# kotoba-tech/kotoba-whisper

Hardware: AMD Instinct MI355X
Metric: audio-seconds/sec (RTF) whisper-large-v3 30s@bs32 (higher is better)
Workload: dtype bf16; 1 GPU; config 3: whisper-large-v3 greedy generate, 30 s clips, log-mel on GPU; model=openai/whisper-large-v3, global_batch=32, per_gpu_batch=32, max_length=128, seq_len=1500, parallelism=dp1

## Files before the change

kotoba-whisper_amd/csrc/decproj.h:

```cpp
#pragma once
#include "declin_tile.h"
#include "kw_common.h"

#ifndef KW_PROJ_STAMP
#define KW_PROJ_STAMP(slot)
#endif

namespace {

constexpr int PROJ_KTM = 5;
constexpr int PROJ_NV = 8;
constexpr int PROJ_SCRATCH = 16384 + 2048 + 256;

struct ProjArgs {
  const bf16_t* x;
  int64_t ldx;
  int M, K, N;
  float ln_eps;
  const float* colsum;
  const bf16x8* W;
  const float* bias;
  float scale;
  int scale_cols;
  int* fault;
};

__host__ __device__ __forceinline__ bool proj_shape_ok(int64_t M, int64_t K) {
  return M >= 1 && M <= 32 && K % 32 == 0 && K / 32 <= PROJ_NV * PROJ_KTM;
}

template <bool ONESHOT>
__device__ __forceinline__ void proj_publish_granules(const ProjArgs& a, int cg, char* scratch,
                                                      unsigned long long* gran) {
  f32x4(*red)[2][64] = reinterpret_cast<f32x4(*)[2][64]>(scratch);
  float(*rpart)[32][2] = reinterpret_cast<float(*)[32][2]>(scratch + 16384);
  float(*rstat)[2] = reinterpret_cast<float(*)[2]>(scratch + 16384 + 2048);
  const int lane = threadIdx.x & 63, wave = __builtin_amdgcn_readfirstlane(threadIdx.x >> 6);
  const int M = a.M, nkt = a.K >> 5;
  const int nv = (nkt + PROJ_KTM - 1) / PROJ_KTM;
  KW_PROJ_STAMP(0);
  const bool xtiled = a.ldx == KW_LD_TILED;
  const int xks = xtiled ? (M > 16 ? 1024 : 512) : 32;
  const bf16_t* x0 = xtiled ? a.x + lane * 8 : a.x + (int64_t)min(lane & 15, M - 1) * a.ldx + (lane >> 4) * 8;
  const bf16_t* x1 = xtiled ? x0 + (M > 16 ? 512 : 0) : a.x + (int64_t)min(16 + (lane & 15), M - 1) * a.ldx + (lane >> 4) * 8;
  const int n_e = min(cg * 16 + (lane & 15), a.N - 1);
  const float ebias = a.bias ? a.bias[n_e] : 0.f;
  const float ecsum = a.colsum[n_e];
  const int fault = __hip_atomic_load(a.fault, __ATOMIC_RELAXED, __HIP_MEMORY_SCOPE_AGENT);
  bf16x8 wv[2][PROJ_KTM];
#pragma unroll
  for (int r = 0; r < 2; ++r) {
    const int v = min(wave + 4 * r, nv - 1);
    const int kt0 = (nkt * v) / nv, kt1 = (nkt * (v + 1)) / nv;
    const int ktl = max(kt1 - 1, kt0);
    if (wave + 4 * r < nv) {
#pragma unroll
      for (int u = 0; u < PROJ_KTM; ++u)
        wv[r][u] = __builtin_nontemporal_load(a.W + ((int64_t)cg * nkt + min(kt0 + u, ktl)) * 64 + lane);
    }
  }
  bf16x8 av[2][2][PROJ_KTM];
  auto load_a = [&](int r) {
    const int v = min(wave + 4 * r, nv - 1);
    const int kt0 = (nkt * v) / nv, kt1 = (nkt * (v + 1)) / nv;
    const int ktl = max(kt1 - 1, kt0);
#pragma unroll
    for (int u = 0; u < PROJ_KTM; ++u) {
      const int kt = min(kt0 + u, ktl);
      av[r][0][u] = *reinterpret_cast<const bf16x8*>(x0 + kt * xks);
      av[r][1][u] = *reinterpret_cast<const bf16x8*>(x1 + kt * xks);
    }
  };
  load_a(0);
  if (ONESHOT && wave + 4 < nv) load_a(1);
#pragma unroll
  for (int r = 0; r < 2; ++r) {
    const int v = wave + 4 * r;
    if (v >= nv) break;
    const int kt0 = (nkt * v) / nv, kt1 = (nkt * (v + 1)) / nv;
    const bf16x8* w = wv[r];
    if (!ONESHOT && r) load_a(1);
    const bf16x8(&a0)[PROJ_KTM] = av[r][0];
    const bf16x8(&a1)[PROJ_KTM] = av[r][1];
    f32x4 c0 = f32x4{0.f, 0.f, 0.f, 0.f}, c1 = c0;
#pragma unroll
    for (int u = 0; u < PROJ_KTM; ++u)
      if (kt0 + u < kt1) {
        c0 = __builtin_amdgcn_mfma_f32_16x16x32_bf16(a0[u], w[u], c0, 0, 0, 0);
        c1 = __builtin_amdgcn_mfma_f32_16x16x32_bf16(a1[u], w[u], c1, 0, 0, 0);
      }
    ln_row_partials<PROJ_KTM, true>(a0, a1, kt0, kt1, lane, rpart[v]);
    red[v][0][lane] = c0;
    red[v][1][lane] = c1;
  }
  KW_PROJ_STAMP(1);
  __syncthreads();
  if (wave >= 2) return;
  const int hh = wave;
  f32x4 c = red[0][hh][lane];
  for (int v = 1; v < nv; ++v) c += red[v][hh][lane];
  if (lane < 16) ln_finish_row(rpart, nv, 16 * hh + lane, a.K, a.ln_eps, rstat);
  wave_lds_sync();
  const int n = cg * 16 + (lane & 15);
  const bool drop = cg == 0 && fault != 0;
  if (drop && wave == 0 && lane == 0) __hip_atomic_store(a.fault, 0, __ATOMIC_RELAXED, __HIP_MEMORY_SCOPE_AGENT);
#pragma unroll
  for (int r = 0; r < 4; ++r) {
    const int m = 16 * hh + 4 * (lane >> 4) + r;
    float v = c[r];
    v = ln_fold(v, rstat[m][0], rstat[m][1], ecsum);
    v += ebias;
    if (n < a.scale_cols) v *= a.scale;
    const uint32_t mine = f2bf(v);
    const uint32_t other = (uint32_t)__builtin_amdgcn_update_dpp(0, (int)mine, 0xB1, 0xF, 0xF, false);
    if ((lane & 1) == 0 && m < M && n < a.N && !drop)
      __hip_atomic_store(gran + (int64_t)m * (a.N / 2) + (n >> 1), (1ull << 32) | (mine | (other << 16)),
                         __ATOMIC_RELAXED, __HIP_MEMORY_SCOPE_AGENT);
  }
  KW_PROJ_STAMP(2);
}

}
```

kotoba-whisper_amd/csrc/qkvself.hip:

```cpp
#include "attn_common.h"
#include "decproj.h"

#ifndef KW_QS_STAMP
#define KW_QS_STAMP(slot)
#endif

namespace {

constexpr int QS_PAIRS = 2;
constexpr int QS_MAX_LEN = 256;

struct QSP {
  const bf16_t* x;
  int64_t ldx;
  float ln_eps;
  const float* ln_colsum;
  const bf16x8* W;
  const float* bias;
  float scale;
  int M, d, H, n_lin;
  bf16_t* kc;
  bf16_t* vc;
  int t_max;
  const int32_t* cur_len;
  unsigned long long* gran;
  int* err;
  bf16_t* out;
  int out_t;
};

__global__ __launch_bounds__(256) __attribute__((amdgpu_waves_per_eu(3))) void qkv_self_kernel(QSP p) {
  __shared__ __attribute__((aligned(16))) char scratch[PROJ_SCRATCH];
  __shared__ float ared[QS_PAIRS][2][64];
  __shared__ float astat[QS_PAIRS][4];
  __shared__ uint32_t stage[QS_PAIRS][96];
  const int d = p.d, H = p.H, M = p.M;
  if ((int)blockIdx.x < p.n_lin) {
    proj_publish_granules<true>(ProjArgs{p.x, p.ldx, M, d, 3 * d, p.ln_eps, p.ln_colsum, p.W, p.bias, p.scale, d, p.err + 1},
                          blockIdx.x, scratch, p.gran);
    return;
  }
  KW_QS_STAMP(4);
  const int tid = threadIdx.x, lane = tid & 63, wave = __builtin_amdgcn_readfirstlane(tid >> 6);
  const int ps = wave >> 1, pw = wave & 1, ptid = tid & 127;
  const int L = *p.cur_len;
  const bool len_ok = L >= 1 && L <= QS_MAX_LEN && L <= p.t_max;
  const int Lc = len_ok ? L : 1;
  const int p0 = Lc - 1;

  const int pair = ((int)blockIdx.x - p.n_lin) * QS_PAIRS + ps;
  const bool has_pair = pair < M * H;
  const int b = has_pair ? pair / H : 0, h = has_pair ? pair - (pair / H) * H : 0;
  const int sub = lane & 7, slot = pw * 8 + (lane >> 3);
  bf16_t* kb = p.kc + ((int64_t)b * H + h) * p.t_max * HD;
  bf16_t* vb = p.vc + ((int64_t)b * H + h) * p.t_max * HD;
  const int nj0 = min((Lc + 15) >> 4, 8), nj1 = max(min((Lc - 128 + 15) >> 4, 8), 0);
  u32x4 kr[8], vr[8];
  if (has_pair) {
#pragma unroll
    for (int j = 0; j < 8; ++j)
      if (j < nj0) kr[j] = ld_row8<bf16_t>(kb + (int64_t)min(slot + 16 * j, p0) * HD + sub * 8).u[0];
#pragma unroll
    for (int j = 0; j < 8; ++j)
      if (j < nj0) vr[j] = ld_row8<bf16_t>(vb + (int64_t)min(slot + 16 * j, p0) * HD + sub * 8).u[0];
  }

  if (has_pair && ptid < 96) {
    const int part = ptid >> 5, c = ptid & 31;
    unsigned long long* g = p.gran + (int64_t)b * (3 * d / 2) + part * (d / 2) + h * 32 + c;
    unsigned long long x = 0;
    int it = 0;
    for (;; ++it) {
      x = __hip_atomic_load(g, __ATOMIC_RELAXED, __HIP_MEMORY_SCOPE_AGENT);
      if ((x >> 32) == 1ull || it >= XG_SPIN_LIMIT) break;
      __builtin_amdgcn_s_sleep(KW_POLL_SLEEP);
    }
    if ((x >> 32) != 1ull || !len_ok) {
      x = 0x7fc07fc0ull;
      __hip_atomic_store(p.err, 1, __ATOMIC_RELAXED, __HIP_MEMORY_SCOPE_AGENT);
    }
    stage[ps][ptid] = (uint32_t)x;
    __hip_atomic_store(g, 0ull, __ATOMIC_RELAXED, __HIP_MEMORY_SCOPE_AGENT);
  }
  __syncthreads();
  KW_QS_STAMP(5);
  if (has_pair) {
    const uint32_t* st = stage[ps];
    const u32x4 qraw = {st[sub * 4], st[sub * 4 + 1], st[sub * 4 + 2], st[sub * 4 + 3]};
    const u32x4 knew = {st[32 + sub * 4], st[32 + sub * 4 + 1], st[32 + sub * 4 + 2], st[32 + sub * 4 + 3]};
    const u32x4 vnew = {st[64 + sub * 4], st[64 + sub * 4 + 1], st[64 + sub * 4 + 2], st[64 + sub * 4 + 3]};
    float ql[8];
    query_log2(qraw, ql);
    const int pn = p0 >> 7, jn = (p0 & 127) >> 4, sn = p0 & 15;
#pragma unroll
    for (int j = 0; j < 8; ++j)
      if (pn == 0 && j == jn && slot == sn) {
        kr[j] = knew;
        vr[j] = vnew;
      }
    float mw, lw, acc[8];
    wave_row_bf16<16>(ql, kr, vr, 0, Lc, slot, nj0, mw, lw, acc);
    if (nj1 > 0) {
#pragma unroll
      for (int j = 0; j < 8; ++j)
        if (j < nj1) kr[j] = ld_row8<bf16_t>(kb + (int64_t)min(128 + slot + 16 * j, p0 - 1) * HD + sub * 8).u[0];
#pragma unroll
      for (int j = 0; j < 8; ++j)
        if (j < nj1) vr[j] = ld_row8<bf16_t>(vb + (int64_t)min(128 + slot + 16 * j, p0 - 1) * HD + sub * 8).u[0];
#pragma unroll
      for (int j = 0; j < 8; ++j)
        if (pn == 1 && j == jn && slot == sn) {
          kr[j] = knew;
          vr[j] = vnew;
        }
      float m1, l1, a1[8];
      wave_row_bf16<16>(ql, kr, vr, 128, Lc, slot, nj1, m1, l1, a1);
      const float mn = fmaxf(mw, m1);
      const float f0 = __builtin_amdgcn_exp2f(mw - mn), f1 = __builtin_amdgcn_exp2f(m1 - mn);
      lw = fmaf(lw, f0, l1 * f1);
#pragma unroll
      for (int i = 0; i < 8; ++i) acc[i] = fmaf(acc[i], f0, a1[i] * f1);
      mw = mn;
    }
    if (slot == sn && len_ok) {
      *reinterpret_cast<u32x4*>(kb + (int64_t)p0 * HD + sub * 8) = knew;
      *reinterpret_cast<u32x4*>(vb + (int64_t)p0 * HD + sub * 8) = vnew;
    }
    if (lane < 8) {
#pragma unroll
      for (int i = 0; i < 8; ++i) ared[ps][pw][lane * 8 + i] = acc[i];
    }
    if (lane == 0) {
      astat[ps][pw] = mw;
      astat[ps][2 + pw] = lw;
    }
  }
  KW_QS_STAMP(6);
  __syncthreads();
  if (has_pair && ptid < HD) {
    const float* st = astat[ps];
    const float m = fmaxf(st[0], st[1]);
    const float f0 = __builtin_amdgcn_exp2f(st[0] - m), f1 = __builtin_amdgcn_exp2f(st[1] - m);
    const float l = fmaf(st[2], f0, st[3] * f1);
    const float o = fmaf(ared[ps][0][ptid], f0, ared[ps][1][ptid] * f1);
    p.out[p.out_t ? kw_tiled_off(b, h * HD + ptid, p.out_t) : (int64_t)b * d + h * HD + ptid] = f2bf(o / l);
  }
  KW_QS_STAMP(7);
}

size_t qs_gran_bytes(int64_t M, int64_t d) { return (size_t)M * (size_t)(3 * d / 2) * sizeof(unsigned long long); }

bool qs_shape_ok(int64_t M, int64_t d, int64_t H) {
  return proj_shape_ok(M, d) && H >= 1 && d == 64 * H;
}

}

extern "C" size_t kw_dec_qkv_self_workspace(int64_t M, int64_t d) {
  return (M >= 1 && d > 0) ? qs_gran_bytes(M, d) + 64 : 0;
}

extern "C" size_t kw_dec_qkv_self_status_offset(int64_t M, int64_t d) {
  return (M >= 1 && d > 0) ? qs_gran_bytes(M, d) : 0;
}

extern "C" int kw_dec_qkv_self_supported(int64_t M, int64_t d, int64_t H) {
  return qs_shape_ok(M, d, H) ? 1 : 0;
}

extern "C" int kw_dec_qkv_self(const kw_dec_qkv_self_args* a, kw_stream_t stream) {
  if (!a || !a->x || !a->W || !a->ln_colsum || !a->k_cache || !a->v_cache || !a->cur_len || !a->out || !a->workspace)
    return kw_set_error_msg(KW_EINVAL, "kw_dec_qkv_self: null pointer");
  if (!qs_shape_ok(a->M, a->d, a->H) || (a->ldx != KW_LD_TILED && (a->ldx < a->d || a->ldx % 8)) || (uintptr_t)a->x % 16 || a->t_max < 1 ||
      a->t_max > 4096)
    return kw_set_error_msg(KW_EINVAL, "kw_dec_qkv_self: M <= 32 rows, d = 64 H <= 1280, ldx % 8 == 0, 16-B aligned x");
  if (a->ws_bytes < kw_dec_qkv_self_workspace(a->M, a->d))
    return kw_set_error_msg(KW_EINVAL, "kw_dec_qkv_self: needs a zero-filled workspace of kw_dec_qkv_self_workspace()");
  QSP p;
  p.x = reinterpret_cast<const bf16_t*>(a->x);
  p.ldx = a->ldx;
  p.ln_eps = a->ln_eps;
  p.ln_colsum = a->ln_colsum;
  p.W = reinterpret_cast<const bf16x8*>(a->W);
  p.bias = a->bias;
  p.scale = a->scale;
  p.M = (int)a->M;
  p.d = (int)a->d;
  p.H = (int)a->H;
  p.n_lin = (int)(3 * a->d / 16);
  p.kc = reinterpret_cast<bf16_t*>(a->k_cache);
  p.vc = reinterpret_cast<bf16_t*>(a->v_cache);
  p.t_max = (int)a->t_max;
  p.cur_len = a->cur_len;
  p.gran = reinterpret_cast<unsigned long long*>(a->workspace);
  p.err = reinterpret_cast<int*>(reinterpret_cast<char*>(a->workspace) + qs_gran_bytes(a->M, a->d));
  p.out = reinterpret_cast<bf16_t*>(a->out);
  p.out_t = a->ldx == KW_LD_TILED ? (int)((a->M + 15) / 16) : 0;
  const int grid = p.n_lin + (int)((a->M * a->H + QS_PAIRS - 1) / QS_PAIRS);
  hipLaunchKernelGGL(qkv_self_kernel, dim3((unsigned)grid), dim3(256), 0, (hipStream_t)stream, p);
  KW_CHECK_LAUNCH();
  return KW_OK;
}
```

Baseline: 2391 audio-s/s.

## Widen qkv_self blocks to 8 waves and stagger attention KV loads

Doubles the attention pairs per block to four, giving 512-thread blocks. Adds a projection variant in which each of eight waves handles one K-slice in a single pass, instead of four waves looping over two slices. Attention blocks now sleep briefly before loading the KV cache, so the projection blocks' weight streaming gets memory bandwidth first. The aim is less serialization inside projection blocks and less contention with the attention prologue. The costs are a fixed sleep on the attention path, lower occupancy from the larger blocks, and tuning that depends on timing.

```diff
diff --git a/kotoba-whisper_amd/csrc/decproj.h b/kotoba-whisper_amd/csrc/decproj.h
--- a/kotoba-whisper_amd/csrc/decproj.h
+++ b/kotoba-whisper_amd/csrc/decproj.h
@@ -120,4 +120,59 @@
   KW_PROJ_STAMP(2);
 }
 
+__device__ __forceinline__ void proj_publish_granules_w8(const ProjArgs& a, int cg, char* scratch,
+                                                         unsigned long long* gran) {
+  f32x4(*red)[2][64] = reinterpret_cast<f32x4(*)[2][64]>(scratch);
+  float(*rpart)[32][2] = reinterpret_cast<float(*)[32][2]>(scratch + 16384);
+  float(*rstat)[2] = reinterpret_cast<float(*)[2]>(scratch + 16384 + 2048);
+  const int lane = threadIdx.x & 63, wave = __builtin_amdgcn_readfirstlane(threadIdx.x >> 6);
+  const int M = a.M, nkt = a.K >> 5;
+  const int nv = (nkt + PROJ_KTM - 1) / PROJ_KTM;
+  KW_PROJ_STAMP(0);
+  const int n_e = min(cg * 16 + (lane & 15), a.N - 1);
+  if (wave < nv) {
+    const int kt0 = (nkt * wave) / nv, kt1 = (nkt * (wave + 1)) / nv;
+    const int ktl = max(kt1 - 1, kt0);
+    bf16x8 w[1][PROJ_KTM], a0[PROJ_KTM], a1[PROJ_KTM];
+    load_w_frags<PROJ_KTM, 1, true>(a.W, cg, nkt, kt0, ktl, lane, w);
+    if (a.ldx == KW_LD_TILED)
+      load_x_frags_tiled<PROJ_KTM, true>(a.x, M > 16 ? 2 : 1, kt0, ktl, lane, a0, a1);
+    else
+      load_x_frags_rows<PROJ_KTM, true>(a.x, a.ldx, M, kt0, ktl, lane, a0, a1);
+    f32x4 c0[1], c1[1];
+    mfma_tile<PROJ_KTM, 1, true>(a0, a1, w, kt0, kt1, c0, c1);
+    ln_row_partials<PROJ_KTM, true>(a0, a1, kt0, kt1, lane, rpart[wave]);
+    red[wave][0][lane] = c0[0];
+    red[wave][1][lane] = c1[0];
+  }
+  const float ebias = a.bias ? a.bias[n_e] : 0.f;
+  const float ecsum = a.colsum[n_e];
+  const int fault = __hip_atomic_load(a.fault, __ATOMIC_RELAXED, __HIP_MEMORY_SCOPE_AGENT);
+  KW_PROJ_STAMP(1);
+  __syncthreads();
+  if (wave >= 2) return;
+  const int hh = wave;
+  f32x4 c = red[0][hh][lane];
+  for (int v = 1; v < nv; ++v) c += red[v][hh][lane];
+  if (lane < 16) ln_finish_row(rpart, nv, 16 * hh + lane, a.K, a.ln_eps, rstat);
+  wave_lds_sync();
+  const int n = cg * 16 + (lane & 15);
+  const bool drop = cg == 0 && fault != 0;
+  if (drop && wave == 0 && lane == 0) __hip_atomic_store(a.fault, 0, __ATOMIC_RELAXED, __HIP_MEMORY_SCOPE_AGENT);
+#pragma unroll
+  for (int r = 0; r < 4; ++r) {
+    const int m = 16 * hh + 4 * (lane >> 4) + r;
+    float v = c[r];
+    v = ln_fold(v, rstat[m][0], rstat[m][1], ecsum);
+    v += ebias;
+    if (n < a.scale_cols) v *= a.scale;
+    const uint32_t mine = f2bf(v);
+    const uint32_t other = (uint32_t)__builtin_amdgcn_update_dpp(0, (int)mine, 0xB1, 0xF, 0xF, false);
+    if ((lane & 1) == 0 && m < M && n < a.N && !drop)
+      __hip_atomic_store(gran + (int64_t)m * (a.N / 2) + (n >> 1), (1ull << 32) | (mine | (other << 16)),
+                         __ATOMIC_RELAXED, __HIP_MEMORY_SCOPE_AGENT);
+  }
+  KW_PROJ_STAMP(2);
 }
+
+}
diff --git a/kotoba-whisper_amd/csrc/qkvself.hip b/kotoba-whisper_amd/csrc/qkvself.hip
--- a/kotoba-whisper_amd/csrc/qkvself.hip
+++ b/kotoba-whisper_amd/csrc/qkvself.hip
@@ -5,9 +5,13 @@
 #define KW_QS_STAMP(slot)
 #endif
 
+#ifndef KW_QS_KV_DELAY
+#define KW_QS_KV_DELAY 48
+#endif
+
 namespace {
 
-constexpr int QS_PAIRS = 2;
+constexpr int QS_PAIRS = 4;
 constexpr int QS_MAX_LEN = 256;
 
 struct QSP {
@@ -29,15 +33,15 @@
   int out_t;
 };
 
-__global__ __launch_bounds__(256) __attribute__((amdgpu_waves_per_eu(3))) void qkv_self_kernel(QSP p) {
+__global__ __launch_bounds__(64 * 2 * QS_PAIRS) __attribute__((amdgpu_waves_per_eu(4))) void qkv_self_kernel(QSP p) {
   __shared__ __attribute__((aligned(16))) char scratch[PROJ_SCRATCH];
   __shared__ float ared[QS_PAIRS][2][64];
   __shared__ float astat[QS_PAIRS][4];
   __shared__ uint32_t stage[QS_PAIRS][96];
   const int d = p.d, H = p.H, M = p.M;
   if ((int)blockIdx.x < p.n_lin) {
-    proj_publish_granules<true>(ProjArgs{p.x, p.ldx, M, d, 3 * d, p.ln_eps, p.ln_colsum, p.W, p.bias, p.scale, d, p.err + 1},
-                          blockIdx.x, scratch, p.gran);
+    proj_publish_granules_w8(ProjArgs{p.x, p.ldx, M, d, 3 * d, p.ln_eps, p.ln_colsum, p.W, p.bias, p.scale, d, p.err + 1},
+                             blockIdx.x, scratch, p.gran);
     return;
   }
   KW_QS_STAMP(4);
@@ -56,6 +60,7 @@
   bf16_t* vb = p.vc + ((int64_t)b * H + h) * p.t_max * HD;
   const int nj0 = min((Lc + 15) >> 4, 8), nj1 = max(min((Lc - 128 + 15) >> 4, 8), 0);
   u32x4 kr[8], vr[8];
+  if (KW_QS_KV_DELAY > 0) __builtin_amdgcn_s_sleep(KW_QS_KV_DELAY);
   if (has_pair) {
 #pragma unroll
     for (int j = 0; j < 8; ++j)
@@ -197,7 +202,7 @@
   p.out = reinterpret_cast<bf16_t*>(a->out);
   p.out_t = a->ldx == KW_LD_TILED ? (int)((a->M + 15) / 16) : 0;
   const int grid = p.n_lin + (int)((a->M * a->H + QS_PAIRS - 1) / QS_PAIRS);
-  hipLaunchKernelGGL(qkv_self_kernel, dim3((unsigned)grid), dim3(256), 0, (hipStream_t)stream, p);
+  hipLaunchKernelGGL(qkv_self_kernel, dim3((unsigned)grid), dim3(64 * 2 * QS_PAIRS), 0, (hipStream_t)stream, p);
   KW_CHECK_LAUNCH();
   return KW_OK;
 }
```

New measurement: 2387 audio-s/s. About the same (-0.2%).
